# PASSIONLab/BELLA

Measured on AMD Instinct MI355X. Metric: candidate overlap pairs/sec, higher is better.
Workload: dtype u16/u32 integer

## Files before the change

bella_amd/api.py:

```python
from __future__ import annotations

import ctypes as C
import os
import dataclasses
import sys

import numpy as np

from . import _lib
from ._lib import CLIP_DT, GraphTrimParams, TrimStats
from ._lib import ALN_DT, CONS_DT, EDGE_DT, EXT_DT, LINK_DT, OVL_DT, PAIR_DT, PLACE_DT, POLISH_DT, PolishParams, PolishStats, RealignParams, RealignStats, BubbleStats, GraphBubbleParams, GraphCleanParams, GraphWeakParams, WeakStats, GraphParams, GraphStats, UnitigStats, PILEUP_COUNTERS, SEED_DT, TRACE_DT, ConsensusParams, Memory, Params, Timings, TraceStats, WriteStats


class BellaHipError(RuntimeError):
    def __init__(self, code, msg):
        super().__init__("bella_hip error %d: %s" % (code, msg))
        self.code = code


@dataclasses.dataclass
class BellaPars:
    kmerSize: int = 17
    binSize: int = 500
    xDrop: int = 7
# ... 191 lines not shown
        nnz = int(rowids_t.numel())
        self._chk(self.lib.bella_hip_set_B_device(self.h, k, nkmers, colptr_t.data_ptr(), rowids_t.data_ptr() if nnz else None,
                                                  values_t.data_ptr() if nnz else None, nnz))

    def get_B(self):
        nnz = C.c_uint64(0)
        self._chk(self.lib.bella_hip_get_B(self.h, C.byref(nnz), None, None, None))
        colptr = np.zeros(self.nreads + 1, np.uint32)
        rowids = np.zeros(max(nnz.value, 1), np.uint32)
        values = np.zeros(max(nnz.value, 1), np.uint16)
        self._chk(self.lib.bella_hip_get_B(self.h, C.byref(nnz), colptr.ctypes.data, rowids.ctypes.data, values.ctypes.data))
        return colptr, rowids[:nnz.value], values[:nnz.value]

    def set_partition(self, first, stride):
        self._chk(self.lib.bella_hip_set_partition(self.h, first, stride))

    def set_column_range(self, first, count):
        self._chk(self.lib.bella_hip_set_column_range(self.h, first, count))

    def set_debug(self, flags):
        self._chk(self.lib.bella_hip_set_debug(self.h, flags))

    TUNE = {"lds_tiers": 0, "kcount_budget": 1, "wide_budget": 2, "xdrop_variant": 3, "row_lists": 4, "xdrop_class_min": 5,
            "layout_order": 6, "inline_entries": 7, "row_path": 8, "cache_bytes": 9, "dist_layout": 10, "compact_b": 11}

    def reserve(self, nbytes: int) -> float:
        ms = C.c_double(0.0)
        self._chk(self.lib.bella_hip_reserve(self.h, int(nbytes), C.byref(ms)))
        return ms.value

    def trim(self):
        self._chk(self.lib.bella_hip_trim(self.h))

    def set_tuning(self, what: str, *values):
        v = np.asarray(values, dtype=np.uint64)
        self._chk(self.lib.bella_hip_set_tuning(self.h, self.TUNE[what], v.ctypes.data if len(v) else None, len(v)))

    def overlap(self, pars: BellaPars):
        n, f = C.c_uint64(0), C.c_uint64(0)
        cp = pars.c()
        self._chk(self.lib.bella_hip_overlap(self.h, C.byref(cp), C.byref(n), C.byref(f)))
        self.npairs, self.flops = n.value, f.value
        return n.value, f.value

    def count_pairs(self, pars: BellaPars):
        n, f = C.c_uint64(0), C.c_uint64(0)
        cp = pars.c()
# ... 470 lines not shown
```

bella_amd/csrc/assemble.hpp:

```cpp
#pragma once
#include <hip/hip_runtime.h>
#include "core.hpp"
#include "slotorder.hpp"
#include "util.hpp"

namespace bella {

__global__ void k_pack_reads(const uint8_t* bases, uint64_t total, uint32_t* packed, uint64_t nwords, uint32_t* status) {
    const uint64_t w = (uint64_t)blockIdx.x * blockDim.x + threadIdx.x;
    if (w >= nwords) return;
    uint32_t out = 0;
    bool bad = false;
    for (uint32_t t = 0; t < 16; ++t) {
        const uint64_t g = w * 16 + t;
        if (g >= total) break;
        const uint32_t c = bases[g];
        uint32_t code;
        switch (c) {
            case 'A': code = 0; break;
            case 'C': code = 1; break;
            case 'G': code = 2; break;
            case 'T': code = 3; break;
            default: code = 0; bad = true;
        }
// ... 458 lines not shown
    if (i < nreads)
        for (uint32_t e = Bloc[i] + lane_id(); e < Bloc[i + 1]; e += 64) { const uint32_t cnt = bent_count(Bent[e], inl); n += cnt ? 1u : 0u; f += cnt; }
#pragma unroll
    for (int d = 32; d > 0; d >>= 1) { n += __shfl_xor(n, d, 64); f += __shfl_xor(f, d, 64); }
    if (lane_id() == 0) {
        if (len) len[i] = n;
        rowF[i] = f;
    }
}
__global__ __launch_bounds__(kBlock) void k_layout_compact(const uint32_t* Bloc, const uint32_t* Bnew, const uint2* Bent, uint32_t nreads, uint32_t inl,
                                                           uint2* out) {
    const uint32_t i = blockIdx.x * kWaves + wave_id();
    if (i >= nreads) return;
    const uint32_t b0 = Bloc[i], b1 = Bloc[i + 1];
    uint32_t o = Bnew[i];
    for (uint32_t e0 = b0; e0 < b1; e0 += 64) {
        const uint32_t e = e0 + lane_id();
        uint2 be = make_uint2(0u, 0u);
        if (e < b1) be = Bent[e];
        const bool live = e < b1 && bent_count(be, inl) != 0;
        const unsigned long long m = __ballot(live);
        if (live) out[o + (uint32_t)__popcll(m & ((1ull << lane_id()) - 1ull))] = be;
        o += (uint32_t)__popcll(m);
    }
}

constexpr int kRowListBlock = 1024;
__global__ __launch_bounds__(kRowListBlock) void k_layout_rowlists(const uint32_t* Bptr, const uint2* Bent, const uint2* Aent, const uint64_t* starts,
                                                                   const uint64_t* roff, const uint32_t* cols, uint32_t nrows, uint2* Aent2, uint16_t* Aov,
                                                                   uint32_t inl) {
    __shared__ uint32_t scr[kRowListBlock / 64];
    __shared__ uint32_t s_off[kRowListBlock];
    __shared__ uint2 s_be[kRowListBlock];
    for (uint32_t x = blockIdx.x; x < nrows; x += gridDim.x) {
        const uint32_t i = cols ? cols[x] : x;
        const uint32_t b0 = Bptr[i], n = Bptr[i + 1] - b0;
        const uint64_t o = starts[x];
        uint64_t running = 0;
        for (uint32_t jb = 0; jb < n; jb += kRowListBlock) {
            const uint32_t j = jb + threadIdx.x;
            const uint32_t nround = n - jb < (uint32_t)kRowListBlock ? n - jb : (uint32_t)kRowListBlock;
            uint2 be = make_uint2(0u, 0u);
            if (j < n) be = Bent[b0 + j];
            const uint32_t cnt = bent_count(be, inl);
            uint32_t tot;
            const uint32_t ex = block_excl_scan<kRowListBlock / 64>(cnt, scr, &tot);
// ... 44 lines not shown
```

bella_amd/csrc/bella_hip.hip:

```cpp
#include <hip/hip_runtime.h>
#include <hipcub/hipcub.hpp>

#include <algorithm>
#include <cmath>
#include <initializer_list>
#include <iterator>
#include <map>
#include <cstdarg>
#include <cstdio>
#include <cstdlib>
#include <chrono>
#include <cstring>
#include <string>
#include <thread>
#include <vector>

#include "../../include/bella_hip.h"
#include "assemble.hpp"
#include "comm.hpp"
#include "core.hpp"
#include "fastq.hpp"
#include "graph.hpp"
#include "trim.hpp"
#include "kcount.hpp"
// ... 197 lines not shown
    uint32_t* pinned = nullptr;
    Stager stager;
    bella_ingest_stats ingest{};
    int caps_state = 0;
    ncclComm_t comm = nullptr;
    const Rccl* api = nullptr;
    int comm_ranks = 0, comm_rank = 0;
    Buf comm_meta;
    bool pass_known = false;
    uint64_t pass_sig[6] = {};
    uint32_t pass_tcnt[20] = {};
    uint64_t pass_products = 0;
    uint64_t pass_wide_products[2] = {};
    bool pass_rare_free = false;
    bool pass_big_free = false;
    uint32_t tier_caps[kNumTiers] = {};
    uint32_t ntiers = 0;
    bool tiers_from_env = false;
    uint64_t kcount_budget = 1ull << 30, wide_budget = 1ull << 30;
    bool lane_order_ok = true;
    uint64_t xdrop_class_min = 4ull * 4096 * 64;
    BufPool pool;
    uint32_t layout_inline = 0;
    uint32_t tune_layout_order = 0;
    uint32_t tune_inline = 0;
    uint32_t tune_row_path = 0;
    uint32_t tune_compact_b = 0;
    uint32_t tune_dist_layout = 2;
    bool dist_agreed = false;
    bool layout_dist = false;
    uint64_t tune_cache_bytes = 192ull << 20;
    uint32_t xdrop_variant = 1;
    size_t lds_attr[24] = {};
    hipStream_t side[kNumTiers + 1]{};
    hipEvent_t fork = nullptr, join[kNumTiers + 1]{};
};

namespace {

int fail(bella_ctx* c, int code, const char* fmt, ...) {
    char b[512];
    va_list ap;
    va_start(ap, fmt);
    vsnprintf(b, sizeof(b), fmt, ap);
    va_end(ap);
    if (c) c->err = b;
    return code;
}

#define HIPCHK(c, call)                                                                                           \
    do {                                                                                                          \
        hipError_t e_ = (call);                                                                                   \
        if (e_ != hipSuccess)                                                                                     \
            return fail(c, BELLA_ERR_HIP, "%s failed: %s (%s:%d)", #call, hipGetErrorString(e_), __FILE__, __LINE__); \
    } while (0)
#define KCHK(c) HIPCHK(c, hipGetLastError())
// ... 240 lines not shown
    }
};

inline const uint32_t* layout_bptr(const bella_ctx* c) { return ptr<uint32_t>(c->Bloc); }

void release_count_scratch(bella_ctx* c) {
    release(c->kc_keys); release(c->kc_alt); release(c->kc_runlen); release(c->kc_flag); release(c->kc_slot);
}

int layout_dist(bella_ctx* c, uint64_t nown_nnz, uint32_t rmask, uint32_t inl, int kbits, uint32_t** ekey_out, uint64_t** eval_out,
                uint32_t** fkey_out, uint64_t** fval_out);
void layout_dist_fail(bella_ctx* c);
bool layout_dist_eligible(const bella_ctx* c);

int build_layout(bella_ctx* c, bool collective = false) {
    release_count_scratch(c);
    const uint64_t nnz = c->nnz;
    const uint32_t nk = c->nkmers;
    const uint32_t pf = c->part_first, ps = c->part_stride;
    if (nnz >= 0xFFFFFFF0ull) return fail(c, BELLA_ERR_BAD_ARG, "nnz(A) must be < 2^32 (KMERINDEX uint32, main.cpp:60)");
    drop(c, MATRIX);
    c->have_rowlists = false;
    c->layout_inline = 0;
    c->tm.expand_ms = 0.f;
    const bool dist = collective && c->dist_agreed;
    struct Bail { bella_ctx* c; bool armed; ~Bail() { if (armed) layout_dist_fail(c); } } bail{c, dist};
    if (dist && (c->debug & 262144u)) return fail(c, BELLA_ERR_STATE, "debug bit 18: this rank fails before its share of the formation");
    if (!dist) {
        ENSURE(c, c->lk_key, 4 * nnz);
        ENSURE(c, c->lk_key2, 4 * nnz);
        ENSURE(c, c->lk_val, 8 * nnz);
        ENSURE(c, c->lk_val2, 8 * nnz);
    }
    ENSURE(c, c->lk_rinfo, 8 * ((size_t)c->nreads + 1));
    ENSURE(c, c->w, 4 * std::max<uint64_t>(nnz + 1, (uint64_t)c->nreads + 2));
    ENSURE(c, c->wscan, 4 * std::max<uint64_t>(nnz + 1, (uint64_t)c->nreads + 2));
    ENSURE(c, c->Aent, 8 * nnz + 64);
    HIPCHK(c, hipMemsetAsync(c->status.p, 0, 4, c->stream));
    HIPCHK(c, hipEventRecord(c->ev[4], c->stream));
    uint64_t nown_nnz = nnz;
    c->layout_first = pf; c->layout_stride = ps;
    ENSURE(c, c->Bloc, 4 * ((size_t)c->nreads + 2));
    if (ps > 1) {
        uint32_t* len = ptr<uint32_t>(c->w);
        k_layout_own_lengths<<<nblk((uint64_t)c->nreads + 1), 256, 0, c->stream>>>(ptr<uint32_t>(c->Bptr), c->nreads, pf, ps, len);
        KCHK(c);
        int rc = scan_u32(c, len, ptr<uint32_t>(c->Bloc), (uint64_t)c->nreads + 1);
        if (rc) return rc;
        uint32_t n32 = 0;
        HIPCHK(c, hipMemcpyAsync(&n32, ptr<uint32_t>(c->Bloc) + c->nreads, 4, hipMemcpyDeviceToHost, c->stream));
        HIPCHK(c, hipStreamSynchronize(c->stream));
        nown_nnz = n32;
    } else {
        HIPCHK(c, hipMemcpyAsync(c->Bloc.p, c->Bptr.p, 4 * ((size_t)c->nreads + 1), hipMemcpyDeviceToDevice, c->stream));
    }
    c->owned_nnz = 0;
    uint32_t ratio1024 = 1024;
    c->long_list_sample = false;
    const uint32_t* Bloc = ptr<uint32_t>(c->Bloc);
    if (c->Bent.cap > 16 * nown_nnz + (1u << 20)) release(c->Bent);
    ENSURE(c, c->Bent, 8 * nown_nnz);
    const bool first_app = c->tune_layout_order == 1 || (c->debug & 1024u);
    c->layout_dist = dist;
    if (nnz || dist) {
        int kbits = 1;
        while (kbits < 32 && (1ull << kbits) < (uint64_t)nk) ++kbits;
        const uint32_t rmask = c->nreads <= (1u << 30) ? 0x3FFFFFFFu : 0x7FFFFFFFu;
        const uint32_t by_kmer = first_app ? 0u : 1u;
        const bool inl_pays = 8ull * nnz > c->tune_cache_bytes || c->tune_inline == 2 || (c->debug & 65536u);
        const uint32_t inl = rmask == 0x3FFFFFFFu && nnz < 0x80000000ull && inl_pays && c->tune_inline != 1 && !(c->debug & 32768u) ? 1u : 0u;
        c->layout_inline = inl;
        uint32_t* ekey = nullptr;
        uint64_t* eval = nullptr;
        const uint32_t* skey = nullptr;
        const uint64_t* sval = nullptr;
        if (dist) {
            uint32_t *fk = nullptr; uint64_t* fv = nullptr;
            bail.armed = false;
            int rcd = layout_dist(c, nown_nnz, rmask, inl, kbits, &ekey, &eval, &fk, &fv);
            if (rcd) return rcd;
// ... 39 lines not shown
            if (rc1) return rc1;
        }
        }
        if (nown_nnz) {
            int ebits = 1;
            while (ebits < 32 && (1ull << ebits) < nown_nnz) ++ebits;
            hipcub::DoubleBuffer<uint32_t> ek(ekey, const_cast<uint32_t*>(skey));
            hipcub::DoubleBuffer<uint64_t> ev(eval, const_cast<uint64_t*>(sval));
            if (ebits > 12) CUB(c, hipcub::DeviceRadixSort::SortPairs, ek, ev, (uint64_t)nown_nnz, ebits - 8, ebits, c->stream);
            k_layout_place<<<((nblk(nown_nnz) + 7u) / 8u) * 8u, 256, 0, c->stream>>>(ek.Current(), ev.Current(), nown_nnz, ptr<uint2>(c->Bent));
            KCHK(c);
        }
        c->owned_nnz = nown_nnz;
        c->live_nnz = nown_nnz;
        ENSURE(c, c->rowF, 4 * ((size_t)c->nreads + 2));
        if (!nown_nnz) HIPCHK(c, hipMemsetAsync(c->rowF.p, 0, 4 * ((size_t)c->nreads + 2), c->stream));
        if (nown_nnz) {
            const bool compact = !c->tune_compact_b;
            uint32_t* len = ptr<uint32_t>(c->w);
            uint32_t* bnew = ptr<uint32_t>(c->wscan);
            k_layout_live<<<nblk((uint64_t)c->nreads + 1, kWaves), kBlock, 0, c->stream>>>(Bloc, ptr<uint2>(c->Bent), c->nreads, inl, compact ? len : nullptr,
                                                                                         ptr<uint32_t>(c->rowF));
            KCHK(c);
            if (compact) {
                int rc = scan_u32(c, len, bnew, (uint64_t)c->nreads + 1);
                if (rc) return rc;
                uint32_t live = 0;
                HIPCHK(c, hipMemcpyAsync(&live, bnew + c->nreads, 4, hipMemcpyDeviceToHost, c->stream));
                HIPCHK(c, hipStreamSynchronize(c->stream));
                TmpBuf out;
                ENSURE(c, out, 8 * (size_t)live);
                k_layout_compact<<<nblk(c->nreads, kWaves), kBlock, 0, c->stream>>>(Bloc, bnew, ptr<uint2>(c->Bent), c->nreads, inl, ptr<uint2>(out));
                if (hipGetLastError() != hipSuccess) return fail(c, BELLA_ERR_HIP, "k_layout_compact failed to launch");
                HIPCHK(c, hipMemcpyAsync(c->Bloc.p, bnew, 4 * ((size_t)c->nreads + 1), hipMemcpyDeviceToDevice, c->stream));
                HIPCHK(c, hipStreamSynchronize(c->stream));
                out.give_to(c->Bent);
                c->live_nnz = live;
            }
        }
        const size_t bitmap_bytes = 4 * (((size_t)c->nreads + 31) / 32);
        uint32_t samp[2] = {0, 0};
        if (c->owned_nnz && bitmap_bytes <= 128 * 1024) {
            HIPCHK(c, hipMemsetAsync(ptr<uint32_t>(c->status) + 6, 0, 16, c->stream));
            const uint32_t ncols = c->nreads / ps + 1;
            const uint32_t nsample = ncols < 512 ? ncols : 512;
            const uint32_t step = (ncols / nsample ? ncols / nsample : 1) * ps;
            HIPCHK(c, hipFuncSetAttribute((const void*)k_sample_pair_ratio, hipFuncAttributeMaxDynamicSharedMemorySize, (int)bitmap_bytes));
            k_sample_pair_ratio<<<nsample, kBlock, bitmap_bytes, c->stream>>>(Bloc, ptr<uint2>(c->Bent), ptr<uint2>(c->Aent),
                                                                             c->nreads, pf, step, ptr<uint32_t>(c->status) + 6, inl);
            KCHK(c);
            HIPCHK(c, hipMemcpyAsync(&ratio1024, ptr<uint32_t>(c->status) + 6, 4, hipMemcpyDeviceToHost, c->stream));
            HIPCHK(c, hipMemcpyAsync(samp, ptr<uint32_t>(c->status) + 8, 8, hipMemcpyDeviceToHost, c->stream));
            HIPCHK(c, hipStreamSynchronize(c->stream));
        }
        c->long_list_sample = samp[1] > 0 && samp[0] <= samp[1];
        const bool auto_lists = c->long_list_sample && !(c->debug & 1u) && c->tune_row_path != 1 && c->lane_order_ok;
        if (by_kmer && (c->want_rowlists || auto_lists) && c->nreads <= (1u << 30)) {
            int rc = ensure_bytes(c, c->Arow, 8 * ((size_t)c->nreads + 2));
            uint64_t F = 0;
            if (!rc) {
                rc = scan_u32_to_u64(c, ptr<uint32_t>(c->rowF), ptr<uint64_t>(c->Arow), (uint64_t)c->nreads + 1);
                if (rc) return rc;
                HIPCHK(c, hipMemcpyAsync(&F, ptr<uint64_t>(c->Arow) + c->nreads, 8, hipMemcpyDeviceToHost, c->stream));
                HIPCHK(c, hipStreamSynchronize(c->stream));
            }
            size_t mfree = 0, mtotal = 0;
            HIPCHK(c, hipMemGetInfo(&mfree, &mtotal));
            mfree += c->pool.bytes + c->pool.arena.largest_hole();
            const bool fits = (double)F * 70.0 + 1e8 <= (double)mfree && !(c->debug & 2048u);
            if (!rc && fits) {
                HIPCHK(c, hipEventRecord(c->ev[10], c->stream));
                rc = ensure_bytes(c, c->Aent2, 8 * F + 64);
                if (!rc) rc = ensure_bytes(c, c->Aov, 2 * F + 64);
                if (!rc) {
                    const uint32_t grid = c->nreads < 4096u ? c->nreads : 4096u;
                    if (grid) k_layout_rowlists<<<grid, kRowListBlock, 0, c->stream>>>(Bloc, ptr<uint2>(c->Bent), ptr<uint2>(c->Aent), ptr<uint64_t>(c->Arow),
                                                                                     ptr<uint64_t>(c->roff), nullptr, c->nreads, ptr<uint2>(c->Aent2), ptr<uint16_t>(c->Aov), inl);
                    KCHK(c);
                    HIPCHK(c, hipEventRecord(c->ev[11], c->stream));
                    HIPCHK(c, hipEventSynchronize(c->ev[11]));
                    c->tm.expand_ms = ev_ms(c->ev[10], c->ev[11]);
                    c->have_rowlists = true;
                }
// ... 173 lines not shown
        case BELLA_TUNE_LAYOUT_ORDER:
            if (n && values[0] > 1) return fail(c, BELLA_ERR_BAD_ARG, "layout order: 0 (k-mer order) or 1 (first appearance)");
            c->tune_layout_order = n ? (uint32_t)values[0] : 0u;
            return 0;
        case BELLA_TUNE_INLINE_ENTRIES:
            if (n && values[0] > 2) return fail(c, BELLA_ERR_BAD_ARG, "inline entries: 0 (by size), 1 (never) or 2 (always)");
            c->tune_inline = n ? (uint32_t)values[0] : 0u;
            return 0;
        case BELLA_TUNE_ROW_PATH:
            if (n && values[0] > 1) return fail(c, BELLA_ERR_BAD_ARG, "row path: 0 (LDS tiers) or 1 (global workspace)");
            c->tune_row_path = n ? (uint32_t)values[0] : 0u;
            c->pass_known = false;
            return 0;
        case BELLA_TUNE_DIST_LAYOUT:
            if (n && values[0] > 2) return fail(c, BELLA_ERR_BAD_ARG, "distributed layout: 0 (never), 1 (always) or 2 (on the in-process transport only)");
            c->tune_dist_layout = n ? (uint32_t)values[0] : 2u;
            return 0;
        case BELLA_TUNE_CACHE_BYTES:
            c->tune_cache_bytes = n && values[0] ? values[0] : (192ull << 20);
            return 0;
        case BELLA_TUNE_COMPACT_B:
            if (n && values[0] > 1) return fail(c, BELLA_ERR_BAD_ARG, "compact B': 0 (drop the entries without a later read) or 1 (keep them)");
            c->tune_compact_b = n ? (uint32_t)values[0] : 0u;
            return 0;
    }
    return fail(c, BELLA_ERR_BAD_ARG, "unknown tuning parameter %u", what);
}

int bella_hip_trim(bella_ctx* c) {
    if (!c) return BELLA_ERR_BAD_ARG;
    HIPCHK(c, hipSetDevice(c->device));
    HIPCHK(c, hipDeviceSynchronize());
    trim_pool(c->pool);
    return 0;
}

int bella_hip_reserve(bella_ctx* c, uint64_t bytes, double* ms) {
    if (!c) return BELLA_ERR_BAD_ARG;
    HIPCHK(c, hipSetDevice(c->device));
    Arena& a = c->pool.arena;
    if (ms) *ms = 0.0;
    if (a.base && a.in_use) return bytes <= a.size ? 0 : fail(c, BELLA_ERR_STATE, "the reserved slab is in use (%zu of %zu bytes)", a.in_use, a.size);
    if (a.base && bytes && bytes <= a.size) return 0;
    if (a.base) { HIPCHK(c, hipDeviceSynchronize()); (void)hipFree(a.base); a = Arena(); }
    if (!bytes) return 0;
    const auto t0 = std::chrono::steady_clock::now();
// ... 1688 lines not shown
        hipStream_t sst = c->stream;
        if (!on_main) {
            const int which = nside;
            int r2 = side_stream(which);
            if (r2) return r2;
            sst = c->side[which];
            nside++;
        }
        a.rowlist = nullptr;
        a.nrows_dev = nullptr;
        a.rowdesc = ptr<uint4>(c->rowlists);
        a.tier_lo = (uint32_t)ln[l].lo;
        a.tier_hi = (uint32_t)ln[l].hi;
        a.tcount_valid = ln[l].hi - ln[l].lo <= 3 ? 1u : 0u;
        for (int k2 = 0; k2 < 4; ++k2) a.tcount[k2] = ln[l].lo + k2 <= ln[l].hi ? tcnt[ln[l].lo + k2] : 0u;
        a.nrows = ln[l].rows;
        a.cap = tier_caps[ln[l].hi];
        a.dcap = dcap_of(a.cap);
        const size_t lds = ln[l].lds;
        const int blk = (c->debug & 8u) ? 512 : kClassBlock[ln[l].cls];
        int ki;
        void (*kern)(SpgemmArgs);
        const bool rl = c->have_rowlists;
#define BELLA_ROWS_KERN(NX, B) (rl ? k_spgemm_rows_lds<NX, B, true> : k_spgemm_rows_lds<NX, B, false>)
        if (blk == 512) {
            ki = a.cap <= 8 * 512 ? 0 : a.cap <= 16 * 512 ? 1 : 2;
            kern = ki == 0 ? BELLA_ROWS_KERN(8, 512) : ki == 1 ? BELLA_ROWS_KERN(16, 512) : BELLA_ROWS_KERN(22, 512);
        } else if (blk == 1024) {
            ki = a.cap <= 4 * 1024 ? 3 : a.cap <= 8 * 1024 ? 4 : 5;
            kern = ki == 3 ? BELLA_ROWS_KERN(4, 1024) : ki == 4 ? BELLA_ROWS_KERN(8, 1024) : BELLA_ROWS_KERN(11, 1024);
        } else if (blk == 256 && a.cap <= 6 * 256) {
            ki = 6;
            kern = BELLA_ROWS_KERN(6, 256);
        } else if (blk == 256) {
            ki = 7;
            kern = BELLA_ROWS_KERN(11, 256);
        } else if (blk == 128) {
            ki = 8;
            kern = BELLA_ROWS_KERN(6, 128);
        } else if (a.cap <= 11 * 64) {
            ki = 18;
            kern = BELLA_ROWS_KERN(11, 64);
        } else {
            ki = 19;
            kern = BELLA_ROWS_KERN(22, 64);
        }
#undef BELLA_ROWS_KERN
        if (rl) ki += ki >= 18 ? 2 : 9;
        if (lds > c->lds_attr[ki]) {
            HIPCHK(c, hipFuncSetAttribute((const void*)kern, hipFuncAttributeMaxDynamicSharedMemorySize, (int)lds));
            c->lds_attr[ki] = lds;
        }
#ifdef BELLA_DEV_PROF
        a.prof = (unsigned long long*)c->prof.p + 10 * l;
        {
            static const int skip = getenv("BELLA_DEV_SKIP_CLASSES") ? atoi(getenv("BELLA_DEV_SKIP_CLASSES")) : 0;
            if (skip & (1 << l)) { a.prof = nullptr; return 0; }
        }
#endif
        kern<<<ln[l].rows, blk, lds, sst>>>(a);
#ifdef BELLA_DEV_PROF
        a.prof = nullptr;
#endif
        KCHK(c);
        launches++;
        return 0;
    };
    c->n_wide = tcnt[g_ntiers] + (mid_to_wide ? n_mid : 0);
    uint32_t* const widelist = (uint32_t*)(ptr<uint4>(c->rowlists) + (size_t)kNumTiers * nr);
    const uint64_t wide_products = c->pass_wide_products[1] + (mid_to_wide ? c->pass_wide_products[0] : 0);
    auto wide_columns = [&]() -> int {
// ... 2428 lines not shown
```

bella_amd/csrc/spgemm.hpp:

```cpp
#pragma once
#include <hip/hip_runtime.h>
#include <type_traits>
#include "../../include/bella_hip.h"
#include "core.hpp"
#include "util.hpp"

namespace bella {

constexpr uint32_t kSU = 4;
constexpr uint32_t kScatterChunk = 64;
#ifndef BELLA_WALK_W
#define BELLA_WALK_W 8
#endif
#ifndef BELLA_GATHER_BATCH
#define BELLA_GATHER_BATCH(blk) 2u
#endif
#ifndef BELLA_SCATTER_CHUNKS
#define BELLA_SCATTER_CHUNKS 8
#endif
#ifndef BELLA_SCATTER_WAVES
#define BELLA_SCATTER_WAVES 1
#endif
#ifndef BELLA_WALK_W_GLOBAL
#define BELLA_WALK_W_GLOBAL 32
// ... 73 lines not shown
    uint32_t* L_gov;
    uint32_t cap, dcap;
};

__device__ __forceinline__ RowMem carve(uint8_t* base, uint32_t cap, uint32_t dcap, bool overlay) {
    RowMem m;
    m.scr = (uint32_t*)base;
    uint32_t* w = (uint32_t*)(base + kRowScratchBytes);
    m.A_hv = w;            w += cap;
    m.A_gov = w;           w += cap;
    m.T1key = w;           w += dcap;
    m.T1cnt = w;           w += dcap;
    m.T1first = w;         w += dcap;
    m.Gaux = w;            w += dcap;
    m.S_p = (uint16_t*)w;  w += (overlay ? 1 : 2) * (((cap + 3) & ~3u) / 2);
    m.M = w;               w += (dcap + 1) / 2;
    if (overlay) { m.L_hv = m.A_hv; m.L_gov = m.A_gov; m.A_fl = nullptr; m.L_fl = nullptr; }
    else { m.L_hv = w; w += cap; m.L_gov = w; w += cap; m.A_fl = (uint8_t*)w; w += (cap + 3) / 4; m.L_fl = (uint8_t*)w; }
    m.cap = cap;
    m.dcap = dcap;
    return m;
}

template <bool OVERLAY, uint32_t NX, int BLK = BELLA_ROW_BLOCK, bool RL = false>
__device__ __forceinline__ bool process_row(const SpgemmArgs& a, const uint32_t i, const uint32_t b0, const uint32_t n, const uint32_t lenV,
                                            const RowMem& m, const uint64_t arow = 0, const uint32_t Fdesc = 0) {
    constexpr int kRowBlock = BLK;
    constexpr int kRowWaves = BLK / 64;
    const uint32_t tid = threadIdx.x;
#ifdef BELLA_DEV_PROF
    long long tc_ = clock64();
#define BELLA_BPROF(n) { const long long t2_ = clock64(); if (tid == 0 && a.prof) atomicAdd(a.prof + (n), (unsigned long long)(t2_ - tc_)); \
                         if (a.stop_phase == (n)) { if (tid == 0) a.nnzC[i] = 0; return true; } tc_ = clock64(); }
#else
#define BELLA_BPROF(n)
#endif
    const uint32_t H1 = m.dcap;
    const uint64_t obase = a.flopptr[__builtin_amdgcn_readfirstlane((int)i)];
    uint32_t* s_chunk = m.scr + 48;
    uint32_t* s_fail = m.scr + 49;
    uint32_t* s_np = m.scr + 50;
    uint32_t* s_nm = m.scr + 51;
    const uint32_t Mcap = (m.dcap + 1) / 2;
    const uint32_t k = (uint32_t)a.k;
    constexpr uint32_t GMASK = OVERLAY ? 0x1FFFu : 0xFFFFu;
    constexpr uint32_t kLastBit = 1u << 29;

#ifndef BELLA_RMAX_SMALL
#define BELLA_RMAX_SMALL 8
#endif
    constexpr uint32_t RMAX = kRowBlock >= 1024 ? 4 : kRowBlock >= 512 ? 8 : BELLA_RMAX_SMALL;
    uint2 be0[RMAX];
    if (!RL) {
        const uint32_t nn = n < RMAX * kRowBlock ? n : RMAX * kRowBlock;
        const uint32_t R = (nn + kRowBlock - 1) / kRowBlock;
        const uint32_t j0 = tid * R;
#pragma unroll
        for (uint32_t u = 0; u < RMAX; ++u) {
            be0[u] = make_uint2(0u, 0u);
            if (u < R && j0 + u < nn) be0[u] = a.Bent[b0 + j0 + u];
        }
    }
    for (uint32_t s = tid; s < H1; s += kRowBlock) { m.T1key[s] = kEmpty; m.T1first[s] = 0; m.T1cnt[s] = 0; }
    if (tid == 0) { *s_chunk = 0; *s_fail = 0; *s_np = 0; *s_nm = 0; }
    __syncthreads();
#ifdef BELLA_DEV_PROF
    { asm volatile("s_waitcnt vmcnt(0)" ::: "memory"); const long long t2_ = clock64(); if (tid == 0 && a.prof) atomicAdd(a.prof + 8, (unsigned long long)(t2_ - tc_)); tc_ = t2_; }
#endif

    uint32_t running = RL ? Fdesc : 0u;
    if (!RL)
    for (uint32_t jb = 0; jb < n; jb += RMAX * kRowBlock) {
        const uint32_t nn = n - jb < RMAX * kRowBlock ? n - jb : RMAX * kRowBlock;
        const uint32_t R = (nn + kRowBlock - 1) / kRowBlock;
        const uint32_t j0 = tid * R;
        uint2 be[RMAX];
        uint32_t csum = 0;
#pragma unroll
        for (uint32_t u = 0; u < RMAX; ++u) {
            be[u] = be0[u];
            if (jb) { be[u] = make_uint2(0u, 0u); if (u < R && j0 + u < nn) be[u] = a.Bent[b0 + jb + j0 + u]; }
            csum += bent_count(be[u], a.inl);
        }
        uint32_t tot;
        uint32_t p = running + block_excl_scan<kRowWaves>(csum, m.scr, &tot);
#pragma unroll
        for (uint32_t u = 0; u < RMAX; ++u) {
            const uint32_t cnt = bent_count(be[u], a.inl);
            for (uint32_t t = 0; t < cnt; ++t) { m.A_hv[p] = be[u].x + t; m.A_gov[p] = be[u].y; ++p; }
        }
        running += tot;
    }
    const uint32_t F = running;
    const uint32_t RB = ((F + 255u) >> 8) << 6;
    __syncthreads();
    BELLA_BPROF(0)
    constexpr uint32_t XB = BELLA_GATHER_BATCH(kRowBlock);
    for (uint32_t base = 0; base < F; base += XB * kRowBlock) {
        uint2 ae[XB];
        uint32_t bw[XB], ax[XB];
        bool inl[XB];
#pragma unroll
        for (uint32_t u = 0; u < XB; ++u) {
            const uint32_t p = base + u * kRowBlock + tid;
            ae[u] = make_uint2(0u, 0u);
            bw[u] = 0; ax[u] = 0;
            inl[u] = false;
            if (p < F) {
                if (RL) { ae[u] = a.Aent2[arow + p]; bw[u] = a.Aov[arow + p]; }
                else {
                    const uint32_t at = m.A_hv[p];
                    bw[u] = m.A_gov[p];
                    inl[u] = a.inl && (at >> 31);
                    ax[u] = at;
                    if (inl[u]) {
                        const uint32_t* ro = (const uint32_t*)a.roff + 2u * (at & 0x3FFFFFFFu);
                        ae[u] = make_uint2(ro[0], ro[2]);
                    } else ae[u] = a.Aent[at];
                }
            }
        }
        uint32_t key[XB], hv[XB], ovf[XB], hh[XB], old[XB];
#pragma unroll
        for (uint32_t u = 0; u < XB; ++u) {
            const uint32_t p = base + u * kRowBlock + tid;
            key[u] = 0; hv[u] = 0; ovf[u] = 0; hh[u] = 0; old[u] = kEmpty;
            if (p >= F) continue;
            uint32_t ov, pal;
            bool oriented;
            if (RL) {
                key[u] = ae[u].x & 0x3FFFFFFFu; pal = (ae[u].x >> 30) & 1u; oriented = (ae[u].x >> 31) != 0; hv[u] = ae[u].y;
                ov = (uint32_t)overlap_estimate(hv[u] & 0xFFFFu, hv[u] >> 16, bw[u], lenV, oriented, k) & 0xFFFFu;
            } else if (inl[u]) {
                key[u] = ax[u] & 0x3FFFFFFFu;
                const uint32_t posH = bw[u] >> 16, posV = bw[u] & 0xFFFFu;
                pal = 0;
                oriented = ((ax[u] >> 30) & 1u) != 0;
                ov = (uint32_t)overlap_estimate(posH, posV, ae[u].y - ae[u].x, lenV, oriented, k) & 0xFFFFu;
                hv[u] = posH | (posV << 16);
            } else {
                key[u] = ae[u].x & 0x7FFFFFFFu;
                const uint32_t posH = ae[u].y & 0xFFFFu, lenH = ae[u].y >> 16;
// ... 7 lines not shown
            hh[u] = hash_range(key[u], H1);
        }
#pragma unroll
        for (uint32_t u = 0; u < XB; ++u)
            if (base + u * kRowBlock + tid < F) old[u] = atomicCAS(&m.T1key[hh[u]], kEmpty, key[u]);
#pragma unroll
        for (uint32_t u = 0; u < XB; ++u) {
            const uint32_t p = base + u * kRowBlock + tid;
            if (p >= F) continue;
            uint32_t h = hh[u], o = old[u];
            uint32_t probes = 0;
            while (o != kEmpty && o != key[u]) {
                if (++probes == H1) break;
                h = (h + 1 == H1) ? 0 : h + 1;
                o = atomicCAS(&m.T1key[h], kEmpty, key[u]);
            }
            if (probes == H1) { *s_fail = 1; continue; }
            const uint32_t q = (p >= RB ? 1u : 0u) + (p >= 2u * RB ? 1u : 0u) + (p >= 3u * RB ? 1u : 0u);
            atomicAdd((q & 2u) ? &m.T1first[h] : &m.T1cnt[h], (q & 1u) ? 0x10000u : 1u);
            m.A_hv[p] = hv[u];
            if (OVERLAY) m.A_gov[p] = (ovf[u] & 0xC000FFFFu) | (h << 16);
            else { m.A_gov[p] = (h << 16) | (ovf[u] & 0xFFFFu); m.A_fl[p] = (uint8_t)(ovf[u] >> 30); }
        }
    }
    __syncthreads();
    BELLA_BPROF(1)
    if (*s_fail) return false;

    uint32_t Fm, d;
    {
        const uint32_t c = (H1 + kRowBlock - 1) / kRowBlock;
        const uint32_t lo = tid * c < H1 ? tid * c : H1;
        const uint32_t hi = lo + c < H1 ? lo + c : H1;
        uint32_t occ = 0, csum = 0;
        for (uint32_t s = lo; s < hi; ++s) {
            const uint32_t w0 = m.T1cnt[s], w1 = m.T1first[s];
            const uint32_t mm = (w0 & 0xFFFFu) + (w0 >> 16) + (w1 & 0xFFFFu) + (w1 >> 16);
            occ += mm ? 1u : 0u;
            csum += mm > 1 ? mm : 0u;
        }
        uint32_t tot;
        const uint32_t ex = block_excl_scan<kRowWaves>((occ << 16) | csum, m.scr, &tot);
        Fm = tot & 0xFFFFu;
        d = tot >> 16;
        uint32_t rank = ex >> 16, st = ex & 0xFFFFu;
        for (uint32_t s = lo; s < hi; ++s) {
// ... 301 lines not shown
        const uint32_t flags = (fl & 1u) | ((((fl & 1u) ^ 1u) | (fl >> 1)) << 1);
        *(uint4*)(a.tmp_pairs + obase + r) = make_uint4(keyw & 0x7FFFFFFFu, firstp, (cw >> 16) | ((hv & 0xFFFFu) << 16), (hv >> 16) | (flags << 16));
        if (a.tmp_ext) {
            bella_pair_ext ex;
            ex.nbins = (uint16_t)nroots; ex.support = (uint16_t)sup; ex.binov = (uint16_t)(m.L_gov[st + win] & 0xFFFFu); ex.pad = 0;
            a.tmp_ext[obase + r] = ex;
        }
    };
    if (dense) {
        for (uint32_t j = tid; j < nm; j += kRowBlock) { const uint32_t mj = m.M[j]; e_one(mj & 0xFFFFu, mj >> 16); }
    } else {
        for (uint32_t g = tid; g < H1; g += kRowBlock)
            if (m.T1key[g] != kEmpty && (m.T1cnt[g] & 0xFFFFu) >= 2u) e_one(g, ((const uint16_t*)m.M)[g]);
    }
    if (tid == 0) a.nnzC[i] = d;
    BELLA_BPROF(7)
#ifdef BELLA_DEV_PROF
    if (tid == 0 && a.prof) atomicAdd(a.prof + 9, 1ull);
#endif
#undef BELLA_BPROF
    return true;
}

template <uint32_t NX, int BLK = BELLA_ROW_BLOCK, bool RL = false>
__global__ __launch_bounds__(BLK, (BLK == 64 ? (NX <= 11 ? 4 : 2) : BLK == 1024 ? (NX <= 4 ? 8 : 4) : BLK <= 256 ? 8 : (NX <= 8 ? 6 : 2))) void k_spgemm_rows_lds(SpgemmArgs a) {
    extern __shared__ __attribute__((aligned(16))) uint8_t smem[];
    uint32_t x = blockIdx.x, t = a.tier_hi;
    if (a.tcount_valid) {
#pragma unroll
        for (int k2 = 3; k2 >= 1; --k2)
            if (a.tier_lo + (uint32_t)k2 == t && x >= a.tcount[k2]) { x -= a.tcount[k2]; --t; }
        const uint32_t rel = t - a.tier_lo;
        const uint32_t ct = rel == 0 ? a.tcount[0] : rel == 1 ? a.tcount[1] : rel == 2 ? a.tcount[2] : a.tcount[3];
        if (x >= ct) return;
    } else {
        const uint32_t* tc = a.ctl + kCtlTierCnt;
        while (t > a.tier_lo && x >= tc[t]) { x -= tc[t]; --t; }
        if (x >= tc[t]) return;
    }
    const uint4 ds = a.rowdesc[(size_t)t * a.nreads + x];
    const uint32_t i = ds.x;
    const RowMem m = carve(smem, a.cap, a.dcap, true);
    const bool ok = RL ? process_row<true, NX, BLK, true>(a, i, 0u, 0u, ds.z >> 16, m, (uint64_t)ds.y | ((uint64_t)(ds.z & 0xFFFFu) << 32), ds.w)
                       : process_row<true, NX, BLK, false>(a, i, ds.y, ds.z & 0xFFFFu, ds.z >> 16, m);
    if (!ok && threadIdx.x == 0) a.retry[atomicAdd(&a.ctl[kCtlRetry], 1u)] = i;
}

#ifndef BELLA_GLOBAL_BLOCK
#define BELLA_GLOBAL_BLOCK 1024
#endif
constexpr int kGlobalBlock = BELLA_GLOBAL_BLOCK;
template <bool RL>
__global__ __launch_bounds__(kGlobalBlock) void k_spgemm_rows_global(SpgemmArgs a) {
    uint8_t* ws = a.ws + (uint64_t)blockIdx.x * a.ws_stride;
    const uint32_t nrows = a.nrows_dev ? *a.nrows_dev : a.nrows;
    for (uint32_t x = blockIdx.x; x < nrows; x += gridDim.x) {
        const uint32_t i = a.rowdesc ? a.rowdesc[x].x : a.rowlist[x];
        uint32_t f = a.flops[i];
        if (f < 16u) f = 16u;
        const RowMem m = carve(ws, f, f, false);
        const uint32_t b0 = a.Bptr[i];
        if (RL) (void)process_row<false, 8, kGlobalBlock, true>(a, i, 0u, 0u, (uint32_t)(a.roff[i + 1] - a.roff[i]), m, a.Arow[i], a.flops[i]);
        else (void)process_row<false, 8, kGlobalBlock, false>(a, i, b0, a.Bptr[i + 1] - b0, (uint32_t)(a.roff[i + 1] - a.roff[i]), m);
        __syncthreads();
    }
}

// ... 158 lines not shown
    if (blockIdx.x == 0 && threadIdx.x < kCtlWords) ctl[threadIdx.x] = 0;
    const uint32_t j = blockIdx.x * blockDim.x + threadIdx.x;
    if (j >= nown) return;
    const uint32_t i = i0 + j * stride;
    nnzC[i] = 0;
    flops[i] = rowF[i];
}

__global__ __launch_bounds__(kBlock) void k_tier_lists(const uint32_t* flops, uint32_t nreads, uint32_t i0, uint32_t stride, uint32_t nown,
                                                       const uint32_t* caps, uint32_t ntiers,
                                                       const uint32_t* Bptr, const uint64_t* roff, uint4* desc, uint32_t* widelist,
                                                       uint32_t* counts, unsigned long long* total, uint64_t* obase, const uint64_t* Arow) {
    const uint32_t j = blockIdx.x * blockDim.x + threadIdx.x;
    const uint32_t i = i0 + j * stride;
    const uint32_t f = j < nown ? flops[i] : 0u;
    uint32_t tier = 0xFFFFFFFFu;
    uint4 ds = make_uint4(i, 0u, 0u, 0u);
    if (f > 0) {
        tier = ntiers;
        for (uint32_t t = 0; t < ntiers; ++t)
            if (f <= caps[t]) { tier = t; break; }
        const uint32_t b0 = Bptr[i];
        ds.y = b0;
        ds.z = (Bptr[i + 1] - b0) | ((uint32_t)(roff[i + 1] - roff[i]) << 16);
        if (Arow) {
            const uint64_t ar = Arow[i];
            ds.y = (uint32_t)ar;
            ds.z = (uint32_t)((ar >> 32) & 0xFFFFu) | ((uint32_t)(roff[i + 1] - roff[i]) << 16);
            ds.w = f;
        }
    }
    __shared__ uint32_t s_cnt[16], s_base[16];
    if (threadIdx.x < 16) s_cnt[threadIdx.x] = 0;
    __syncthreads();
    {
        unsigned long long inc = f;
#pragma unroll
        for (int dlt = 1; dlt < 64; dlt <<= 1) {
            const unsigned long long t = __shfl_up(inc, dlt, 64);
            if ((int)lane_id() >= dlt) inc += t;
        }
        const unsigned long long tot = __shfl(inc, 63, 64);
        unsigned long long base = 0;
        if (lane_id() == 0 && tot) base = atomicAdd(total, tot);
        base = __shfl(base, 0, 64);
        if (j < nown) obase[i] = base + inc - f;
        if (__ballot(tier + 1 >= ntiers && tier != 0xFFFFFFFFu)) {
// ... 66 lines not shown
```

include/bella_hip.h:

```cpp
#ifndef BELLA_HIP_H
#define BELLA_HIP_H

#include <stddef.h>
#include <stdint.h>

#ifdef __cplusplus
extern "C" {
#endif

#define BELLA_HIP_ABI_VERSION 6

enum {
    BELLA_OK = 0,
    BELLA_ERR_NO_DEVICE = -1,
    BELLA_ERR_HIP = -2,
    BELLA_ERR_BAD_ARG = -3,
    BELLA_ERR_BAD_BASE = -4,
    BELLA_ERR_READ_TOO_LONG = -5,
    BELLA_ERR_TUPLE_ORDER = -6,
    BELLA_ERR_STATE = -7,
    BELLA_ERR_ROW_TOO_LARGE = -8,
    BELLA_ERR_BINS = -9,
    BELLA_ERR_NOMEM = -10
};
// ... 432 lines not shown
int bella_hip_allgather_panels(bella_ctx* ctx);
int bella_hip_count_kmers_dist(bella_ctx* ctx, uint16_t kmer_size, uint32_t lower, uint32_t upper, uint32_t selector, uint32_t window,
                               uint32_t first_read, uint32_t nreads_block, uint32_t* nkmers, uint64_t* ntuples, uint64_t* ndistinct);

int bella_hip_get_timings(bella_ctx* ctx, bella_timings* t);
typedef struct {
    uint64_t reads_bytes;
    uint64_t matrix_bytes;
    uint64_t layout_A_bytes;
    uint64_t layout_B_bytes;
    uint64_t rowlist_bytes;
    uint64_t pass_bytes;
    uint64_t other_bytes;
    uint64_t owned_nnz;
    uint64_t layout_shared;
    uint64_t live_nnz;
} bella_memory;
int bella_hip_get_memory(bella_ctx* ctx, bella_memory* m);
int bella_hip_get_memory_sized(bella_ctx* ctx, void* m, uint64_t struct_size);
int bella_hip_set_debug(bella_ctx* ctx, uint32_t flags);
int bella_hip_reserve(bella_ctx* ctx, uint64_t bytes, double* ms);
int bella_hip_trim(bella_ctx* ctx);
enum { BELLA_TUNE_LDS_TIERS = 0, BELLA_TUNE_KCOUNT_BUDGET = 1, BELLA_TUNE_WIDE_BUDGET = 2, BELLA_TUNE_XDROP_VARIANT = 3, BELLA_TUNE_ROW_LISTS = 4,
       BELLA_TUNE_XDROP_CLASS_MIN = 5, BELLA_TUNE_LAYOUT_ORDER = 6, BELLA_TUNE_INLINE_ENTRIES = 7, BELLA_TUNE_ROW_PATH = 8, BELLA_TUNE_CACHE_BYTES = 9, BELLA_TUNE_DIST_LAYOUT = 10, BELLA_TUNE_COMPACT_B = 11 };
int bella_hip_set_tuning(bella_ctx* ctx, uint32_t what, const uint64_t* values, uint32_t n);

#ifdef __cplusplus
}
#endif
#endif
```

Baseline: 12.78 billion.

## Expand B' into one entry per product so SpGEMM rows skip expansion

Adds an optional layout in which each compacted B' entry is pre-expanded into one entry per product, with offsets and counts rewritten per product. A new PE variant of the LDS row kernel then streams these entries straight into the hash phase, preloading them into registers and skipping the per-row expansion loop and one barrier. It is chosen automatically when row lists are off and B' exceeds the cache budget, provided the expanded size stays within 1.5x the nnz bytes. The cost is a larger B' array and an extra layout kernel and scan. It also adds a tuning knob to force or disable the path.

```diff
diff --git a/bella_amd/api.py b/bella_amd/api.py
--- a/bella_amd/api.py
+++ b/bella_amd/api.py
@@ -237,7 +237,7 @@
         self._chk(self.lib.bella_hip_set_debug(self.h, flags))
 
     TUNE = {"lds_tiers": 0, "kcount_budget": 1, "wide_budget": 2, "xdrop_variant": 3, "row_lists": 4, "xdrop_class_min": 5,
-            "layout_order": 6, "inline_entries": 7, "row_path": 8, "cache_bytes": 9, "dist_layout": 10, "compact_b": 11}
+            "layout_order": 6, "inline_entries": 7, "row_path": 8, "cache_bytes": 9, "dist_layout": 10, "compact_b": 11, "product_entries": 12}
 
     def reserve(self, nbytes: int) -> float:
         ms = C.c_double(0.0)
diff --git a/bella_amd/csrc/assemble.hpp b/bella_amd/csrc/assemble.hpp
--- a/bella_amd/csrc/assemble.hpp
+++ b/bella_amd/csrc/assemble.hpp
@@ -504,6 +504,45 @@
         const unsigned long long m = __ballot(live);
         if (live) out[o + (uint32_t)__popcll(m & ((1ull << lane_id()) - 1ull))] = be;
         o += (uint32_t)__popcll(m);
+    }
+}
+
+__global__ __launch_bounds__(64) void k_layout_compact_products(const uint32_t* Bloc, const uint64_t* start, uint32_t* Bnew, const uint2* Bent,
+                                                                uint32_t nreads, uint32_t inl, uint2* out) {
+    __shared__ uint32_t s_ex[64];
+    __shared__ uint2 s_be[64];
+    const uint32_t i = blockIdx.x;
+    if (i >= nreads) return;
+    const uint32_t b0 = Bloc[i], b1 = Bloc[i + 1];
+    const uint32_t lane = threadIdx.x;
+    uint32_t o = (uint32_t)start[i];
+    if (lane == 0) { Bnew[i] = o; if (i + 1 == nreads) Bnew[nreads] = (uint32_t)start[nreads]; }
+    for (uint32_t e0 = b0; e0 < b1; e0 += 64) {
+        const uint32_t e = e0 + lane;
+        uint2 be = make_uint2(0u, 0u);
+        if (e < b1) be = Bent[e];
+        const uint32_t cnt = e < b1 ? bent_count(be, inl) : 0u;
+        const uint32_t inc = wave_incl_scan(cnt);
+        const uint32_t T = (uint32_t)__builtin_amdgcn_readlane((int)inc, 63);
+        if ((uint32_t)__popcll(__ballot(cnt != 0)) == T) {
+            if (cnt) out[o + inc - 1] = bent_is_inline(be, inl) ? be : make_uint2(be.x, (be.y & 0xC000FFFFu) | 0x10000u);
+            o += T;
+            continue;
+        }
+        __syncthreads();
+        s_ex[lane] = inc - cnt;
+        s_be[lane] = be;
+        __syncthreads();
+        for (uint32_t q = lane; q < T; q += 64) {
+            uint32_t j = 0;
+#pragma unroll
+            for (uint32_t step = 32; step > 0; step >>= 1)
+                if (s_ex[j + step] <= q) j += step;
+            const uint2 sb = s_be[j];
+            const uint32_t t = q - s_ex[j];
+            out[o + q] = bent_is_inline(sb, inl) ? sb : make_uint2(sb.x + t, (sb.y & 0xC000FFFFu) | 0x10000u);
+        }
+        o += T;
     }
 }
 
diff --git a/bella_amd/csrc/bella_hip.hip b/bella_amd/csrc/bella_hip.hip
--- a/bella_amd/csrc/bella_hip.hip
+++ b/bella_amd/csrc/bella_hip.hip
@@ -243,16 +243,18 @@
     uint64_t xdrop_class_min = 4ull * 4096 * 64;
     BufPool pool;
     uint32_t layout_inline = 0;
+    bool layout_products = false;
     uint32_t tune_layout_order = 0;
     uint32_t tune_inline = 0;
     uint32_t tune_row_path = 0;
     uint32_t tune_compact_b = 0;
+    uint32_t tune_product_entries = 0;
     uint32_t tune_dist_layout = 2;
     bool dist_agreed = false;
     bool layout_dist = false;
     uint64_t tune_cache_bytes = 192ull << 20;
     uint32_t xdrop_variant = 1;
-    size_t lds_attr[24] = {};
+    size_t lds_attr[40] = {};
     hipStream_t side[kNumTiers + 1]{};
     hipEvent_t fork = nullptr, join[kNumTiers + 1]{};
 };
@@ -539,6 +541,8 @@
     drop(c, MATRIX);
     c->have_rowlists = false;
     c->layout_inline = 0;
+    c->layout_products = false;
+    c->live_nnz = 0;
     c->tm.expand_ms = 0.f;
     const bool dist = collective && c->dist_agreed;
     struct Bail { bella_ctx* c; bool armed; ~Bail() { if (armed) layout_dist_fail(c); } } bail{c, dist};
@@ -573,6 +577,8 @@
     }
     c->owned_nnz = 0;
     uint32_t ratio1024 = 1024;
+    uint64_t rowF_total = 0;
+    bool rowF_scanned = false;
     c->long_list_sample = false;
     const uint32_t* Bloc = ptr<uint32_t>(c->Bloc);
     if (c->Bent.cap > 16 * nown_nnz + (1u << 20)) release(c->Bent);
@@ -658,12 +664,40 @@
             k_layout_live<<<nblk((uint64_t)c->nreads + 1, kWaves), kBlock, 0, c->stream>>>(Bloc, ptr<uint2>(c->Bent), c->nreads, inl, compact ? len : nullptr,
                                                                                          ptr<uint32_t>(c->rowF));
             KCHK(c);
+            uint32_t live = 0;
             if (compact) {
                 int rc = scan_u32(c, len, bnew, (uint64_t)c->nreads + 1);
                 if (rc) return rc;
-                uint32_t live = 0;
                 HIPCHK(c, hipMemcpyAsync(&live, bnew + c->nreads, 4, hipMemcpyDeviceToHost, c->stream));
-                HIPCHK(c, hipStreamSynchronize(c->stream));
+            }
+            const bool ask_products = compact && c->tune_product_entries != 1 &&
+                                      (c->tune_product_entries == 2 || (!c->want_rowlists && 8ull * nnz > c->tune_cache_bytes));
+            if (ask_products) {
+                int rc = scan_u32_to_u64(c, ptr<uint32_t>(c->rowF), ptr<uint64_t>(c->lk_rinfo), (uint64_t)c->nreads + 1);
+                if (rc) return rc;
+                HIPCHK(c, hipMemcpyAsync(&rowF_total, ptr<uint64_t>(c->lk_rinfo) + c->nreads, 8, hipMemcpyDeviceToHost, c->stream));
+                rowF_scanned = true;
+            }
+            if (compact) HIPCHK(c, hipStreamSynchronize(c->stream));
+            if (ask_products) {
+                Buf& start = c->lk_rinfo;
+                const uint64_t F = rowF_total;
+                const bool small = 8ull * F <= 12ull * nown_nnz || c->tune_product_entries == 2;
+                if (F && F < 0xFFFFFFF0ull && small && !(c->debug & 2048u)) {
+                    TmpBuf out;
+                    if (!ensure_bytes(c, out, 8 * (size_t)F)) {
+                        k_layout_compact_products<<<c->nreads, 64, 0, c->stream>>>(Bloc, ptr<uint64_t>(start), bnew, ptr<uint2>(c->Bent), c->nreads, inl,
+                                                                                   ptr<uint2>(out));
+                        if (hipGetLastError() != hipSuccess) return fail(c, BELLA_ERR_HIP, "k_layout_compact_products failed to launch");
+                        HIPCHK(c, hipMemcpyAsync(c->Bloc.p, bnew, 4 * ((size_t)c->nreads + 1), hipMemcpyDeviceToDevice, c->stream));
+                        HIPCHK(c, hipStreamSynchronize(c->stream));
+                        out.give_to(c->Bent);
+                        c->live_nnz = F;
+                        c->layout_products = true;
+                    } else c->err.clear();
+                }
+            }
+            if (compact && !c->layout_products) {
                 TmpBuf out;
                 ENSURE(c, out, 8 * (size_t)live);
                 k_layout_compact<<<nblk(c->nreads, kWaves), kBlock, 0, c->stream>>>(Bloc, bnew, ptr<uint2>(c->Bent), c->nreads, inl, ptr<uint2>(out));
@@ -694,7 +728,10 @@
         if (by_kmer && (c->want_rowlists || auto_lists) && c->nreads <= (1u << 30)) {
             int rc = ensure_bytes(c, c->Arow, 8 * ((size_t)c->nreads + 2));
             uint64_t F = 0;
-            if (!rc) {
+            if (!rc && rowF_scanned) {
+                HIPCHK(c, hipMemcpyAsync(c->Arow.p, c->lk_rinfo.p, 8 * ((size_t)c->nreads + 1), hipMemcpyDeviceToDevice, c->stream));
+                F = rowF_total;
+            } else if (!rc) {
                 rc = scan_u32_to_u64(c, ptr<uint32_t>(c->rowF), ptr<uint64_t>(c->Arow), (uint64_t)c->nreads + 1);
                 if (rc) return rc;
                 HIPCHK(c, hipMemcpyAsync(&F, ptr<uint64_t>(c->Arow) + c->nreads, 8, hipMemcpyDeviceToHost, c->stream));
@@ -914,6 +951,11 @@
         case BELLA_TUNE_COMPACT_B:
             if (n && values[0] > 1) return fail(c, BELLA_ERR_BAD_ARG, "compact B': 0 (drop the entries without a later read) or 1 (keep them)");
             c->tune_compact_b = n ? (uint32_t)values[0] : 0u;
+            return 0;
+        case BELLA_TUNE_PRODUCT_ENTRIES:
+            if (n && values[0] > 2) return fail(c, BELLA_ERR_BAD_ARG, "product entries: 0 (by size), 1 (never) or 2 (always)");
+            c->tune_product_entries = n ? (uint32_t)values[0] : 0u;
+            c->pass_known = false;
             return 0;
     }
     return fail(c, BELLA_ERR_BAD_ARG, "unknown tuning parameter %u", what);
@@ -2648,7 +2690,8 @@
         int ki;
         void (*kern)(SpgemmArgs);
         const bool rl = c->have_rowlists;
-#define BELLA_ROWS_KERN(NX, B) (rl ? k_spgemm_rows_lds<NX, B, true> : k_spgemm_rows_lds<NX, B, false>)
+        const bool pe = c->layout_products && !rl;
+#define BELLA_ROWS_KERN(NX, B) (rl ? k_spgemm_rows_lds<NX, B, true> : pe ? k_spgemm_rows_lds<NX, B, false, true> : k_spgemm_rows_lds<NX, B, false>)
         if (blk == 512) {
             ki = a.cap <= 8 * 512 ? 0 : a.cap <= 16 * 512 ? 1 : 2;
             kern = ki == 0 ? BELLA_ROWS_KERN(8, 512) : ki == 1 ? BELLA_ROWS_KERN(16, 512) : BELLA_ROWS_KERN(22, 512);
@@ -2673,6 +2716,7 @@
         }
 #undef BELLA_ROWS_KERN
         if (rl) ki += ki >= 18 ? 2 : 9;
+        else if (pe) ki += ki >= 18 ? 13 : 22;
         if (lds > c->lds_attr[ki]) {
             HIPCHK(c, hipFuncSetAttribute((const void*)kern, hipFuncAttributeMaxDynamicSharedMemorySize, (int)lds));
             c->lds_attr[ki] = lds;
diff --git a/bella_amd/csrc/spgemm.hpp b/bella_amd/csrc/spgemm.hpp
--- a/bella_amd/csrc/spgemm.hpp
+++ b/bella_amd/csrc/spgemm.hpp
@@ -119,7 +119,7 @@
     return m;
 }
 
-template <bool OVERLAY, uint32_t NX, int BLK = BELLA_ROW_BLOCK, bool RL = false>
+template <bool OVERLAY, uint32_t NX, int BLK = BELLA_ROW_BLOCK, bool RL = false, bool PE = false>
 __device__ __forceinline__ bool process_row(const SpgemmArgs& a, const uint32_t i, const uint32_t b0, const uint32_t n, const uint32_t lenV,
                                             const RowMem& m, const uint64_t arow = 0, const uint32_t Fdesc = 0) {
     constexpr int kRowBlock = BLK;
@@ -146,9 +146,34 @@
 #ifndef BELLA_RMAX_SMALL
 #define BELLA_RMAX_SMALL 8
 #endif
+    static_assert(!(PE && RL), "the row lists replace B' in the pass");
+    constexpr uint32_t XB = BELLA_GATHER_BATCH(kRowBlock);
     constexpr uint32_t RMAX = kRowBlock >= 1024 ? 4 : kRowBlock >= 512 ? 8 : BELLA_RMAX_SMALL;
     uint2 be0[RMAX];
-    if (!RL) {
+    uint2 itn[XB];
+#ifndef BELLA_PE_HEAD
+#define BELLA_PE_HEAD 1
+#endif
+#ifndef BELLA_PE_HEAD_MAX
+#define BELLA_PE_HEAD_MAX 8
+#endif
+    constexpr bool HEAD = PE && BELLA_PE_HEAD != 0 && NX <= BELLA_PE_HEAD_MAX;
+    uint2 ith[HEAD ? NX : 1];
+    if (HEAD) {
+#pragma unroll
+        for (uint32_t u = 0; u < NX; ++u) {
+            const uint32_t p = u * kRowBlock + tid;
+            ith[u] = make_uint2(0u, 0u);
+            if (p < n) ith[u] = a.Bent[b0 + p];
+        }
+    } else if (PE) {
+#pragma unroll
+        for (uint32_t u = 0; u < XB; ++u) {
+            const uint32_t p = u * kRowBlock + tid;
+            itn[u] = make_uint2(0u, 0u);
+            if (p < n) itn[u] = a.Bent[b0 + p];
+        }
+    } else if (!RL) {
         const uint32_t nn = n < RMAX * kRowBlock ? n : RMAX * kRowBlock;
         const uint32_t R = (nn + kRowBlock - 1) / kRowBlock;
         const uint32_t j0 = tid * R;
@@ -165,8 +190,8 @@
     { asm volatile("s_waitcnt vmcnt(0)" ::: "memory"); const long long t2_ = clock64(); if (tid == 0 && a.prof) atomicAdd(a.prof + 8, (unsigned long long)(t2_ - tc_)); tc_ = t2_; }
 #endif
 
-    uint32_t running = RL ? Fdesc : 0u;
-    if (!RL)
+    uint32_t running = RL ? Fdesc : PE ? n : 0u;
+    if (!RL && !PE)
     for (uint32_t jb = 0; jb < n; jb += RMAX * kRowBlock) {
         const uint32_t nn = n - jb < RMAX * kRowBlock ? n - jb : RMAX * kRowBlock;
         const uint32_t R = (nn + kRowBlock - 1) / kRowBlock;
@@ -190,10 +215,9 @@
     }
     const uint32_t F = running;
     const uint32_t RB = ((F + 255u) >> 8) << 6;
-    __syncthreads();
+    if (!PE) __syncthreads();
     BELLA_BPROF(0)
-    constexpr uint32_t XB = BELLA_GATHER_BATCH(kRowBlock);
-    for (uint32_t base = 0; base < F; base += XB * kRowBlock) {
+    auto x3_batch = [&](const uint32_t base, const uint2 (&it)[XB]) __attribute__((always_inline)) {
         uint2 ae[XB];
         uint32_t bw[XB], ax[XB];
         bool inl[XB];
@@ -206,8 +230,8 @@
             if (p < F) {
                 if (RL) { ae[u] = a.Aent2[arow + p]; bw[u] = a.Aov[arow + p]; }
                 else {
-                    const uint32_t at = m.A_hv[p];
-                    bw[u] = m.A_gov[p];
+                    const uint32_t at = PE ? it[u].x : m.A_hv[p];
+                    bw[u] = PE ? it[u].y : m.A_gov[p];
                     inl[u] = a.inl && (at >> 31);
                     ax[u] = at;
                     if (inl[u]) {
@@ -215,6 +239,13 @@
                         ae[u] = make_uint2(ro[0], ro[2]);
                     } else ae[u] = a.Aent[at];
                 }
+            }
+        }
+        if (PE && !HEAD) {
+#pragma unroll
+            for (uint32_t u = 0; u < XB; ++u) {
+                const uint32_t p = base + (XB + u) * kRowBlock + tid;
+                if (p < F) itn[u] = a.Bent[b0 + p];
             }
         }
         uint32_t key[XB], hv[XB], ovf[XB], hh[XB], old[XB];
@@ -268,6 +299,24 @@
             if (OVERLAY) m.A_gov[p] = (ovf[u] & 0xC000FFFFu) | (h << 16);
             else { m.A_gov[p] = (h << 16) | (ovf[u] & 0xFFFFu); m.A_fl[p] = (uint8_t)(ovf[u] >> 30); }
         }
+    };
+    if (HEAD) {
+        constexpr uint32_t NB = (NX + XB - 1) / XB;
+#pragma unroll
+        for (uint32_t b = 0; b < NB; ++b) {
+            if (b * XB * kRowBlock >= F) break;
+            uint2 it[XB];
+#pragma unroll
+            for (uint32_t u = 0; u < XB; ++u) it[u] = b * XB + u < NX ? ith[(b * XB + u) % (HEAD ? NX : 1)] : make_uint2(0u, 0u);
+            x3_batch(b * XB * kRowBlock, it);
+        }
+    } else {
+        for (uint32_t base = 0; base < F; base += XB * kRowBlock) {
+            uint2 it[XB];
+#pragma unroll
+            for (uint32_t u = 0; u < XB; ++u) it[u] = PE ? itn[u] : make_uint2(0u, 0u);
+            x3_batch(base, it);
+        }
     }
     __syncthreads();
     BELLA_BPROF(1)
@@ -615,7 +664,7 @@
     return true;
 }
 
-template <uint32_t NX, int BLK = BELLA_ROW_BLOCK, bool RL = false>
+template <uint32_t NX, int BLK = BELLA_ROW_BLOCK, bool RL = false, bool PE = false>
 __global__ __launch_bounds__(BLK, (BLK == 64 ? (NX <= 11 ? 4 : 2) : BLK == 1024 ? (NX <= 4 ? 8 : 4) : BLK <= 256 ? 8 : (NX <= 8 ? 6 : 2))) void k_spgemm_rows_lds(SpgemmArgs a) {
     extern __shared__ __attribute__((aligned(16))) uint8_t smem[];
     uint32_t x = blockIdx.x, t = a.tier_hi;
@@ -635,7 +684,7 @@
     const uint32_t i = ds.x;
     const RowMem m = carve(smem, a.cap, a.dcap, true);
     const bool ok = RL ? process_row<true, NX, BLK, true>(a, i, 0u, 0u, ds.z >> 16, m, (uint64_t)ds.y | ((uint64_t)(ds.z & 0xFFFFu) << 32), ds.w)
-                       : process_row<true, NX, BLK, false>(a, i, ds.y, ds.z & 0xFFFFu, ds.z >> 16, m);
+                       : process_row<true, NX, BLK, false, PE>(a, i, ds.y, ds.z & 0xFFFFu, ds.z >> 16, m);
     if (!ok && threadIdx.x == 0) a.retry[atomicAdd(&a.ctl[kCtlRetry], 1u)] = i;
 }
 
@@ -840,7 +889,7 @@
             if (f <= caps[t]) { tier = t; break; }
         const uint32_t b0 = Bptr[i];
         ds.y = b0;
-        ds.z = (Bptr[i + 1] - b0) | ((uint32_t)(roff[i + 1] - roff[i]) << 16);
+        ds.z = ((Bptr[i + 1] - b0) & 0xFFFFu) | ((uint32_t)(roff[i + 1] - roff[i]) << 16);
         if (Arow) {
             const uint64_t ar = Arow[i];
             ds.y = (uint32_t)ar;
diff --git a/include/bella_hip.h b/include/bella_hip.h
--- a/include/bella_hip.h
+++ b/include/bella_hip.h
@@ -478,7 +478,8 @@
 int bella_hip_reserve(bella_ctx* ctx, uint64_t bytes, double* ms);
 int bella_hip_trim(bella_ctx* ctx);
 enum { BELLA_TUNE_LDS_TIERS = 0, BELLA_TUNE_KCOUNT_BUDGET = 1, BELLA_TUNE_WIDE_BUDGET = 2, BELLA_TUNE_XDROP_VARIANT = 3, BELLA_TUNE_ROW_LISTS = 4,
-       BELLA_TUNE_XDROP_CLASS_MIN = 5, BELLA_TUNE_LAYOUT_ORDER = 6, BELLA_TUNE_INLINE_ENTRIES = 7, BELLA_TUNE_ROW_PATH = 8, BELLA_TUNE_CACHE_BYTES = 9, BELLA_TUNE_DIST_LAYOUT = 10, BELLA_TUNE_COMPACT_B = 11 };
+       BELLA_TUNE_XDROP_CLASS_MIN = 5, BELLA_TUNE_LAYOUT_ORDER = 6, BELLA_TUNE_INLINE_ENTRIES = 7, BELLA_TUNE_ROW_PATH = 8, BELLA_TUNE_CACHE_BYTES = 9, BELLA_TUNE_DIST_LAYOUT = 10, BELLA_TUNE_COMPACT_B = 11,
+       BELLA_TUNE_PRODUCT_ENTRIES = 12 };
 int bella_hip_set_tuning(bella_ctx* ctx, uint32_t what, const uint64_t* values, uint32_t n);
 
 #ifdef __cplusplus
```

Result: faster. 13.41 billion, median of 6 (+4.9%).
